# KumarRobotics/top_down_renderer

Hardware: AMD Instinct MI355X
Metric: particle-updates/sec (render+score+resample) (higher is better)
Workload: dtype f32

## Files before the change

### include/tdr.h

```cpp
#ifndef TDR_H_
#define TDR_H_

#include <stddef.h>
#include <stdint.h>

#ifdef __cplusplus
extern "C" {
#endif

#define TDR_OK 0
#define TDR_ERR_ARG (-1)
#define TDR_ERR_HIP (-2)
#define TDR_ERR_NOMEM (-3)

#define TDR_MAX_CLASSES 15
#define TDR_ST_FIELDS 7
enum { TDR_ST_INIT_X = 0, TDR_ST_INIT_Y = 1, TDR_ST_DX = 2, TDR_ST_DY = 3, TDR_ST_THETA = 4, TDR_ST_SCALE = 5,
       TDR_ST_HAVE_INIT = 6 };

typedef struct tdr_state {
  float init_x_px, init_y_px, dx_m, dy_m, theta, scale;
  uint8_t have_init;
  uint8_t pad_[3];
} tdr_state;
// ... 191 lines not shown
                          int64_t src_shard, float* dst, int64_t dst_cap, const float* info, float* out12, void* stream);

int tdr_config_compact(int on);
int tdr_config_shift_uniform(int mode);
float tdr_config_shift_uniform_span(float cells);
int tdr_config_ray_split(int k);
int tdr_config_cart_skip(int on);
int tdr_config_init_mfma(int on);
int tdr_config_uw_waves(int on);
int64_t tdr_shift_uniform_launches(void);

int tdr_profile_enable(int on);
int tdr_profile_score_ms(double* total_ms, int64_t* launches);
int tdr_profile_shares(double* dense_ms, double* scattered_ms, int64_t* scattered_particles);
int tdr_profile_variants(int64_t out[16]);

int64_t tdr_config_tuning(const char* name, int64_t value);
int tdr_su_tail_plan(int nchunks, int k, int q, int row, int* group, int* s0, int* s1);
size_t tdr_k_su_order_workspace_ints(int64_t n, int nb);
int64_t tdr_k_su_order_slots(int64_t n, int nb);
int tdr_k_su_order(const float* st, int64_t cap, int64_t n, const int32_t* perm, int nb, float span, int32_t* workspace,
                   int32_t* slots_out, int32_t* keys_out, int32_t* counts_out, int* bucket_out, void* stream);
int tdr_k_score_prep(const tdr_map_desc* map, const float* tab, const float* scan_pk, int nb, int nr, float res,
                     const float* st, int64_t cap, int64_t n, int64_t n_total, const int32_t* perm, float uniform_scale,
                     float span, float* workspace, tdr_score_ctx* ctx, int64_t* layout, void* const* out, void* stream);
int tdr_selftest_score(void);
int tdr_k_selftest_round(const float* x, int64_t n, float limit, int32_t* out, void* stream);
int tdr_libm_variant(void);
int tdr_libm_force_variant(int variant);
int tdr_sincosf_host(const float* x, int64_t n, int variant, float* sin_out, float* cos_out);
// ... 307 lines not shown
```

### top_down_renderer_amd/_lib.py

```python
import ctypes as C
import os

_PKG = os.path.dirname(os.path.abspath(__file__))
SO_PATH = os.environ.get("TDR_LIB_PATH") or os.path.join(_PKG, "libtdr_hip.so")

TDR_ST_FIELDS = 7
TDR_MAX_CLASSES = 15
TDR_SVG_NO_KEY = 0xFFFFFFFF


class FilterParamsC(C.Structure):
    _fields_ = [
        ("pos_cov", C.c_float), ("theta_cov", C.c_float), ("regularization", C.c_float),
        ("init_pos_px_x", C.c_float), ("init_pos_px_y", C.c_float), ("init_pos_px_cov", C.c_float),
        ("init_pos_m_x", C.c_float), ("init_pos_m_y", C.c_float),
        ("init_pos_deg_theta", C.c_float), ("init_pos_deg_cov", C.c_float),
        ("force_on_map", C.c_int32),
        ("fixed_scale", C.c_float), ("scale_log_min", C.c_float), ("scale_log_max", C.c_float),
        ("num_classes", C.c_int32),
        ("class_weights", C.c_float * 16),
    ]


class MapDescC(C.Structure):
# ... 142 lines not shown
    "tdr_rng_set_state_host": (_i, [_vp, _vp]),
    "tdr_k_resample_dev": (_i, [_vp, _i64, _i64, _vp, _i64, _i64, _vp, _vp]),
    "tdr_score_ctx_create": (_i, [C.POINTER(_vp)]),
    "tdr_score_ctx_destroy": (None, [_vp]),
    "tdr_score_ctx_span": (C.c_float, [_vp]),
    "tdr_score_ctx_trial_calls": (_i64, [_vp]),
    "tdr_config_tuning": (_i64, [C.c_char_p, _i64]),
    "tdr_su_tail_plan": (_i, [_i, _i, _i, _i, C.POINTER(_i), C.POINTER(_i), C.POINTER(_i)]),
    "tdr_k_su_order_workspace_ints": (C.c_size_t, [_i64, _i]),
    "tdr_k_su_order_slots": (_i64, [_i64, _i]),
    "tdr_k_su_order": (_i, [_vp, _i64, _i64, _vp, _i, _f, _vp, _vp, _vp, _vp, C.POINTER(_i), _vp]),
    "tdr_k_score_prep": (_i, [_vp, _vp, _vp, _i, _i, _f, _vp, _i64, _i64, _i64, _vp, _f, _f, _vp, _vp, C.POINTER(_i64),
                              C.POINTER(_vp), _vp]),
    "tdr_selftest_score": (_i, []),
    "tdr_profile_variants": (_i, [C.POINTER(_i64)]),
    "tdr_score_ctx_set_polar_factors": (_i, [_vp, _vp, _i, _i]),
    "tdr_polar_factors_host": (_i, [_i, _i, _f, _f, _vp]),
    "tdr_k_score_polar_ctx": (_i, [C.POINTER(MapDescC), _vp, _vp, _i, _i, _f, C.POINTER(FilterParamsC), _vp, _i64, _i64,
                                   _i64, _vp, _f, _i, _vp, _vp, _vp, _vp]),
    "tdr_score_geo_workspace_floats": (C.c_size_t, [_i, _i, _i, _i64, _i64]),
    "tdr_k_score_polar_geo": (_i, [C.POINTER(MapDescC), C.POINTER(MapDescC), _vp, _vp, _vp, _f, _f, _i, _i, _f,
                                   C.POINTER(FilterParamsC), _vp, _i64, _i64, _i64, _vp, _f, _i, _vp, _vp, _vp]),
    "tdr_score_cart_workspace_floats": (C.c_size_t, [_i, _i, _i, _i64, _i64]),
    "tdr_k_score_cart": (_i, [C.POINTER(MapDescC), _vp, _i, _i, _f, C.POINTER(FilterParamsC), _vp, _i64, _i64, _i64,
                              _vp, _vp, _vp, _vp]),
    "tdr_score_cart_init_workspace_floats": (C.c_size_t, [_i, _i, _i, _i64, _i64]),
    "tdr_k_score_cart_init": (_i, [C.POINTER(MapDescC), _vp, _i, _i, _f, C.POINTER(FilterParamsC), _vp, _i64, _i64, _i64,
                                   _vp, _vp]),
    "tdr_k_propagate": (_i, [_vp, _i64, _i64, _vp, _f, _f, _f, _i, _f, _f, _vp, _u64, _u64, _i64, _vp]),
    "tdr_rng_create": (_vp, [_u32]),
# ... 195 lines not shown
```

### top_down_renderer_amd/csrc/tdr_common.h

```cpp
#ifndef TDR_COMMON_H_
#define TDR_COMMON_H_
#include <hip/hip_runtime.h>

#include <cmath>
#include <cstdarg>
#include <cstdint>
#include <cstdio>
#include <cstdlib>
#include <cstring>
#include <limits>
#include <type_traits>
#include <utility>
#include <vector>

#include "tdr.h"
#include "tdr_config.h"
#include "tdr_internal.h"

#ifndef TDR_SCORE_U
#define TDR_SCORE_U 4
#endif
#ifndef TDR_INIT_SCAN_LDS
#define TDR_INIT_SCAN_LDS 1
#endif
// ... 43 lines not shown
#define INI_TILE 2048
#define INI_MAX_TILES 2048
int tdr_chain_total(const float* raw, const float* mean_dev, int kind, int64_t n, float* total_out, void* workspace,
                    bool have_sums, hipStream_t st);
struct UwExact {
  float sum, mean, bsum, pad;
};
int tdr_uw_chunk_pass1(const float* raw, int64_t n, void* workspace, int* cnt_valid, hipStream_t st);
int tdr_uw_chunk_pass2(const float* raw, int64_t n, UwExact* ex, const int* cnt_valid, void* workspace, int* cnt_under,
                       hipStream_t st);
int tdr_uw_small(const float* raw, const float* last_dist, int64_t n, float* w, float* info, hipStream_t st);
int tdr_mt_raw_stream(const uint32_t* state, int64_t nblocks, uint32_t* raw, hipStream_t s);
int tdr_mt_advance(const uint32_t* raw, int64_t nblocks, const uint32_t* consumed, uint32_t* state, hipStream_t s);
__host__ __device__ inline bool tdr_has_kslot(int ncls, int rf) { return ncls + 2 <= rf; }
uint32_t* tdr_profile_stats_ptr();
#endif
```

### top_down_renderer_amd/csrc/tdr_score.hip

```cpp

#include "tdr_common.h"
#include "tdr_batch.h"
#include "tdr_sincosf.h"

struct ScoreArgs {
  const float* rec;
  int rows, cols;
  float resolution;
  const float* tab;
  const float* utab = nullptr;
  const float* scan_pk;
  int nb, nr;
  float res;
  const float* st;
  int64_t cap, n;
  const int32_t* order;
  const int32_t* count = nullptr;
  const int32_t* slot_base = nullptr;
  int use_theta_override = 0;
  float theta_override = 0.f;
  int only_uninit = 0;
  int group, nchunks;
  int64_t npad;
  float* part;
// ... 770 lines not shown
  if (!g_variant_stats) {
    if (hipMalloc((void**)&g_variant_stats, 16 * sizeof(uint32_t)) != hipSuccess) { g_variant_stats = nullptr; return nullptr; }
    (void)hipMemset(g_variant_stats, 0, 16 * sizeof(uint32_t));
  }
  return g_variant_stats;
}
extern "C" int tdr_profile_variants(int64_t out[16]) {
  if (!out) return fail(TDR_ERR_ARG, "profile_variants: null pointer");
  for (int k = 0; k < 16; k++) out[k] = 0;
  if (!g_variant_stats) return TDR_OK;
  uint32_t h[16];
  HIP_TRY(hipDeviceSynchronize());
  HIP_TRY(hipMemcpy(h, g_variant_stats, sizeof(h), hipMemcpyDeviceToHost));
  HIP_TRY(hipMemset(g_variant_stats, 0, sizeof(h)));
  for (int k = 0; k < 16; k++) out[k] = h[k];
  return TDR_OK;
}
extern "C" int tdr_profile_enable(int on) {
  g_prof_on = on != 0;
  g_prof_variants = on == 2;
  g_prof_used = 0;
  g_share_valid = false;
  return TDR_OK;
}
extern "C" int tdr_profile_shares(double* dense_ms, double* scattered_ms, int64_t* scattered_particles) {
  if (!dense_ms || !scattered_ms || !scattered_particles) return fail(TDR_ERR_ARG, "profile_shares: null pointer");
  if (!g_share_valid || !g_share_counts) return fail(TDR_ERR_ARG, "profile_shares: no integer-form launch was profiled");
  float ms[2] = {0.f, 0.f};
  for (int k = 0; k < 2; k++) {
    HIP_TRY(hipEventSynchronize(g_share_ev[k][1]));
// ... 592 lines not shown
```

### top_down_renderer_amd/csrc/tdr_score_ray.hip

```cpp
#include "tdr_score_dev.h"
#include "tdr_score_su.h"

int64_t tdr_ray_padded_samples(int nb, int nr) { return (int64_t)nb * ray_blocks(nr, false) * ray_gq(nr, false) * 64; }

struct RayArgs {
  const uint32_t* crec;
  unsigned planes_off;
  unsigned plane_bytes;
  unsigned cmask_off;
  int pkcol;
  const uint32_t* dict_int;
  int dict_n;
  int rows, cols;
  float resolution;
  const float* tab;
  const float* tab_ray;
  const float* fac;
  const float* rad_ray;
  float uscale;
  const uint16_t* desc_ray;
  const uint32_t* list;
  const int32_t* n_list;
  const float* scan_pk;
  int rf, ncls, nb, nr, blocks;
  float res;
  const float* st;
  int64_t cap;
  const int32_t* slots;
  const int32_t* counts;
  const int32_t* inexact;
  int nsplit;
  int64_t npad;
  uint32_t* part;
};

template <int GQ, bool USCALE, bool FAC, bool BM, bool PATCH>
__device__ __forceinline__ void ray_body(const RayArgs& a, unsigned long long* lacc, uint32_t* ldict, uint4* lut, float2* ldir) {
  static_assert(!BM || GQ == 1, "block-major: one step per row");
  static_assert(!PATCH || BM, "the patch order is a block-major order");
  const int nsparse = a.counts[1];
  if ((int64_t)blockIdx.x * 4 >= (int64_t)nsparse * a.nsplit) return;
  const int lane = threadIdx.x & 63, wave = __builtin_amdgcn_readfirstlane(threadIdx.x >> 6);
  for (int t = threadIdx.x; t < a.dict_n; t += 256) ldict[t] = a.dict_int[t];
  if constexpr (PATCH && FAC)
    for (int t = threadIdx.x; t < a.nb; t += 256) ldir[t] = reinterpret_cast<const float2*>(a.fac)[t];
  const unsigned pconst = (unsigned)(a.pkcol + 16) + 128u;
  if (threadIdx.x < 16) {
    const int code = threadIdx.x;
    uint4 e;
    if (code >= 1 && code <= a.ncls) {
      e.x = a.planes_off + (unsigned)(code - 1) * a.plane_bytes + pconst;
      e.y = 0; e.z = 15; e.w = (unsigned)code * 512u;
    } else {
      e.x = a.cmask_off + pconst;
      e.y = 2; e.z = 0; e.w = 0;
    }
    lut[code] = e;
  }
  unsigned long long* const my = lacc + (size_t)wave * (a.ncls + 1) * 64 + lane;
  for (int c = 0; c <= a.ncls; c++) my[c * 64] = 0;
  __syncthreads();
  const int64_t gw = (int64_t)blockIdx.x * 4 + wave;
  const int64_t q = gw / a.nsplit;
  const int part_id = (int)(gw - q * a.nsplit);
  if (q >= nsparse) return;
  const int64_t slot = (int64_t)a.counts[0] + q;
  const int64_t p = a.slots[slot];
  const float scale = a.st[TDR_ST_SCALE * a.cap + p];
  const float fscale = USCALE ? a.uscale : scale;
  const float cx = a.st[TDR_ST_DX * a.cap + p] * scale + a.st[TDR_ST_INIT_X * a.cap + p];
  const float cy = a.st[TDR_ST_DY * a.cap + p] * scale + a.st[TDR_ST_INIT_Y * a.cap + p];
  const float off0 = cy / a.resolution;
  const float off1 = cx / a.resolution;
  const int shift = rot_shift_dev(a.st[TDR_ST_THETA * a.cap + p], a.nb);
  const float rmaxf = (float)a.rows, cmaxf = (float)a.cols;
  const char* __restrict__ crecb = reinterpret_cast<const char*>(a.crec);
  typedef float tdr_v2f __attribute__((ext_vector_type(2)));
  const tdr_v2f offv = {off0, off1};
  auto cell = [&](float tx, float ty, int& ri, int& ci) {
    tdr_v2f pv = {tx, ty};
// ... 82 lines not shown
    }
    uint32_t v[N * GQ], shb[N * GQ], cnt[N * GQ], acc_at[N * GQ];
#pragma unroll
    for (int u = 0; u < N; u++)
#pragma unroll
      for (int g = 0; g < GQ; g++) {
        const int s = u * GQ + g;
        int ri, ci;
        if constexpr (FAC) cell_fac(dir[u], rr_[u][g], ri, ci);
        else cell(tt[u][2 * g], tt[u][2 * g + 1], ri, ci);
        issue(dd[u][g], ri, ci, v[s], shb[s], cnt[s], acc_at[s]);
      }
#pragma unroll
    for (int s = 0; s < N * GQ; s++) consume(v[s], shb[s], cnt[s], acc_at[s]);
  };
  if constexpr (PATCH) {
    const int ngroups = a.nb / RAY_PG, sectors_all = a.blocks * ngroups;
    const int sper = (sectors_all + a.nsplit - 1) / a.nsplit;
    const int s0 = part_id * sper, s1 = min(sectors_all, s0 + sper);
    const int pl_d = lane >> 4, pl_r = lane & (RAY_PR - 1);
    const uint2* __restrict__ descq = reinterpret_cast<const uint2*>(a.desc_ray);
    float rad4[4] = {0.f, 0.f, 0.f, 0.f};
    int cur_seg = -1;
    int seg = s0 / ngroups, pg = s0 - seg * ngroups;
    for (int sc = s0; sc < s1; sc++) {
      if (seg != cur_seg) {
        cur_seg = seg;
#pragma unroll
        for (int qq = 0; qq < 4; qq++) {
          const int j = (seg * 4 + qq) * RAY_PR + pl_r;
          rad4[qq] = j < a.nr ? a.fac[2 * a.nb + j] : 1.0e30f;
        }
      }
      int wi[4];
      tdr_v2f wdir[4];
#pragma unroll
      for (int k = 0; k < 4; k++) {
        int i = pg * RAY_PG + 4 * k + pl_d - shift;
        i += i < 0 ? a.nb : 0;
        wi[k] = i;
        if constexpr (FAC) {
          const float2 dv = ldir[i];
          wdir[k] = (tdr_v2f){dv.x, dv.y};
        }
      }
#pragma unroll
      for (int h = 0; h < 2; h++) {
        uint2 dd[2];
#pragma unroll
        for (int u = 0; u < 2; u++) dd[u] = descq[((int64_t)(seg * 4 + 2 * h + u) * ngroups + pg) * 64 + lane];
        uint32_t v[8], shb[8], cnt[8], acc_at[8];
#pragma unroll
        for (int u = 0; u < 2; u++)
#pragma unroll
          for (int k = 0; k < 4; k++) {
            int ri, ci;
            if constexpr (FAC) {
              cell_fac(wdir[k], rad4[2 * h + u], ri, ci);
            } else {
              const int j = min((seg * 4 + 2 * h + u) * RAY_PR + pl_r, a.nr - 1);
              const int64_t kk = (int64_t)j * a.nb + wi[k];
              if ((seg * 4 + 2 * h + u) * RAY_PR + pl_r < a.nr) cell(a.tab[2 * kk], a.tab[2 * kk + 1], ri, ci);
              else cell(-1.0e30f, -1.0e30f, ri, ci);
            }
            const uint32_t w = k < 2 ? dd[u].x : dd[u].y;
            issue((k & 1) ? (w >> 16) : (w & 0xFFFFu), ri, ci, v[u * 4 + k], shb[u * 4 + k], cnt[u * 4 + k], acc_at[u * 4 + k]);
          }
#pragma unroll
        for (int t = 0; t < 8; t++) consume(v[t], shb[t], cnt[t], acc_at[t]);
      }
      pg++;
      if (pg == ngroups) { pg = 0; seg++; }
    }
  } else {
// ... 15 lines not shown
      cell(a.tab[2 * k], a.tab[2 * k + 1], ri, ci);
      const unsigned cell_off = plane_offset(ri, ci, a.pkcol, (int)(a.planes_off + pconst));
      uint32_t kbit = 0;
      for (int c = 0; c < a.ncls; c++) {
        const float s = a.scan_pk[bin * a.rf + c];
        if (s != 0.f) {
          const uint32_t vv = *reinterpret_cast<const uint16_t*>(crecb + cell_off + (unsigned)c * a.plane_bytes);
          kbit = vv >> 15;
          __hip_atomic_fetch_add(&my[(c + 1) * 64], (unsigned long long)(uint32_t)s * ldict[(vv & 0xFFCu) >> 2],
                                 __ATOMIC_RELAXED, __HIP_MEMORY_SCOPE_WORKGROUP);
        }
      }
      norm += (uint32_t)a.scan_pk[bin * a.rf + a.rf - 1] & (0u - kbit);
    }
  }
  uint32_t* o = a.part + (int64_t)part_id * (2 * a.ncls + 2) * a.npad + slot;
  for (int c = 0; c < a.ncls; c++) {
    unsigned long long s = __hip_atomic_load(&my[(c + 1) * 64], __ATOMIC_RELAXED, __HIP_MEMORY_SCOPE_WORKGROUP);
#pragma unroll
    for (int dlt = 32; dlt > 0; dlt >>= 1) s += __shfl_xor(s, dlt, 64);
    if (lane == 0) {
      o[(int64_t)(2 * c) * a.npad] = (uint32_t)s;
      o[(int64_t)(2 * c + 1) * a.npad] = (uint32_t)(s >> 32);
    }
  }
#pragma unroll
  for (int dlt = 32; dlt > 0; dlt >>= 1) {
    known += __shfl_xor(known, dlt, 64);
    norm += __shfl_xor(norm, dlt, 64);
  }
  if (lane == 0) {
    o[(int64_t)(2 * a.ncls) * a.npad] = norm;
    o[(int64_t)(2 * a.ncls + 1) * a.npad] = known;
  }
}
TDR_TL_BUFFER(g_timeline_ray, tdr_debug_read_timeline_ray)
template <int GQ, bool USCALE, bool BM = false, bool PATCH = false>
__global__ __launch_bounds__(256) void score_polar_ray_kernel(RayArgs a) {
  extern __shared__ unsigned long long lacc[];
  __shared__ uint32_t ldict[TDR_CMAP_MAX_DICT];
  __shared__ uint4 lut[16];
  __shared__ float2 ldir[PATCH ? RAY_PATCH_MAX_NB : 1];
  if (int_form_off(a.inexact)) return;
#ifdef TDR_SCORE_TIMELINE
  if ((int64_t)blockIdx.x * 4 >= (int64_t)a.counts[1] * a.nsplit) return;
#endif
  TDR_TL_BEGIN(g_timeline_ray)
  if (a.fac && a.inexact[2] == 0) ray_body<GQ, USCALE, true, BM, PATCH>(a, lacc, ldict, lut, ldir);
  else ray_body<GQ, USCALE, false, BM, PATCH>(a, lacc, ldict, lut, ldir);
  TDR_TL_END(g_timeline_ray)
}



bool tdr_ray_map_ok(const tdr_map_desc* map) {
  return map->crec && map->dict && map->cwords == tdr_cmap_words(map->ncls) && map->dict_n > 0 &&
         map->dict_n <= TDR_CMAP_MAX_DICT && tdr_cmap_plane_words(map->ncls, map->rows, map->cols) != 0;
}
int tdr_ray_splits(int nb, int nr, int64_t n, bool bm) {
  if (tdr_cfg().ray_split > 0) return tdr_cfg().ray_split;
  const int64_t rows = (int64_t)nb * ray_blocks(nr, bm);
  int s = 1;
  while (s < TDR_RAY_MAX_SPLIT && n * s < 32768 && rows / (2 * s) >= 8) s *= 2;
  if (s == 1 && rows >= 128) s = 2;
// ... 21 lines not shown
  r.fac = L.fac;
  r.rad_ray = reinterpret_cast<const float*>(base + W.ray_rad);
  r.uscale = L.uscale;
  r.desc_ray = reinterpret_cast<const uint16_t*>(base + W.ray_desc);
  r.list = reinterpret_cast<const uint32_t*>(base + W.ray_multi);
  r.n_list = ints + 3;
  r.scan_pk = L.scan_pk;
  r.rf = L.rf; r.ncls = map->ncls; r.nb = L.nb; r.nr = L.nr; r.blocks = ray_blocks(L.nr, ray_bm(L)); r.res = L.res;
  r.st = L.st; r.cap = L.cap;
  r.slots = base + W.slots;
  r.counts = ints;
  r.inexact = ints + 4;
  r.nsplit = L.ray_split;
  r.npad = L.npad;
  r.part = reinterpret_cast<uint32_t*>(L.part);
  const dim3 grid((unsigned)cdiv(L.n * r.nsplit, 4)), block(256);
  const size_t lds = (size_t)4 * (map->ncls + 1) * 64 * sizeof(unsigned long long);
#define TDR_LAUNCH_RAY(GQ)                                                                            \
  if (L.uniform_scale) hipLaunchKernelGGL((score_polar_ray_kernel<GQ, true>), grid, block, lds, s, r); \
  else hipLaunchKernelGGL((score_polar_ray_kernel<GQ, false>), grid, block, lds, s, r);
  if (ray_patch(L)) {
    if (L.uniform_scale) hipLaunchKernelGGL((score_polar_ray_kernel<1, true, true, true>), grid, block, lds, s, r);
    else hipLaunchKernelGGL((score_polar_ray_kernel<1, false, true, true>), grid, block, lds, s, r);
  } else if (ray_bm(L)) {
    if (L.uniform_scale) hipLaunchKernelGGL((score_polar_ray_kernel<1, true, true>), grid, block, lds, s, r);
    else hipLaunchKernelGGL((score_polar_ray_kernel<1, false, true>), grid, block, lds, s, r);
  } else switch (ray_gq(L.nr, false)) {
    case 1: TDR_LAUNCH_RAY(1) break;
    case 2: TDR_LAUNCH_RAY(2) break;
    default: TDR_LAUNCH_RAY(4) break;
  }
#undef TDR_LAUNCH_RAY
// ... 4 lines not shown
```

### top_down_renderer_amd/csrc/tdr_score_su.h

```cpp
#ifndef TDR_SCORE_SU_H_
#define TDR_SCORE_SU_H_
#include "tdr_common.h"

static inline int64_t su_npad(int64_t n, int nb) { return cdiv(n + 63 * std::min<int64_t>(nb, n), 64) * 64; }
bool tdr_su_shape_ok(int nb, int nr, int group, int64_t n_total);
struct SuWs {
  int64_t tab_su, desc, bbox, keys_in, keys_out, vals_in, vals_out, ints, slots, sort_tmp, ray_tab, ray_desc, ray_multi, ray_rad, total;
  int64_t seg_hist;
};
#define TDR_SU_TAIL_INTS 10
#define TDR_RAY_MAX_SPLIT 8
SuWs tdr_su_ws(int nb, int nr, int group, int64_t n);

#define TDR_SU_NSECT 8
__host__ __device__ static inline int su_tail_plan(int nchunks, int k, int q, int row, int* group, int* s0, int* s1) {
  const int lq = q >= 8 ? 3 : (q >= 4 ? 2 : (q >= 2 ? 1 : 0));
  const int kk = k < 0 ? 0 : (k > nchunks ? nchunks : k);
  const int head = nchunks - kk, rows = head + (kk << lq);
  if (row < 0 || row >= rows) return rows;
  if (row < head) {
    *group = row; *s0 = 0; *s1 = TDR_SU_NSECT;
  } else {
    const int t = row - head, part = t & ((1 << lq) - 1);
    *group = head + (t >> lq);
// ... 39 lines not shown
  float best = 16.f;
  float round_best = 16.f, best_ms = 3.0e38f;
  hipEvent_t e0 = nullptr, e1 = nullptr;
  bool open = false, pending = false;
  int64_t trial_calls = 0;
};
float tdr_su_span_begin(SpanTuner* t, int64_t shape, hipStream_t s);
void tdr_su_span_end(SpanTuner* t, hipStream_t s);
int tdr_su_score(const SuLaunch& L, const SuWs& W, hipStream_t s);
bool tdr_ray_map_ok(const tdr_map_desc* map);
int64_t tdr_ray_padded_samples(int nb, int nr);
int tdr_ray_splits(int nb, int nr, int64_t n, bool block_major = false);
#define RAY_PR 16
#define RAY_PG 16
#define RAY_PATCH_MAX_NB 256
static inline bool ray_bm(const SuLaunch& L) { return tdr_cfg().ray_block_major && L.fac != nullptr; }
static inline bool ray_patch(const SuLaunch& L) { return ray_bm(L) && tdr_cfg().ray_patch && L.nb % RAY_PG == 0 && L.nb <= RAY_PATCH_MAX_NB; }
static inline int ray_gq(int nr, bool bm) { return bm ? 1 : (nr <= 64 ? 1 : (nr <= 128 ? 2 : 4)); }
static inline int ray_blocks(int nr, bool bm) { return (int)cdiv(nr, 64 * ray_gq(nr, bm)); }
int tdr_ray_score(const SuLaunch& L, const SuWs& W, hipStream_t s);
#endif
```

### top_down_renderer_amd/csrc/tdr_score_su.hip

```cpp
#include <rocprim/device/device_radix_sort.hpp>

#include <atomic>

#include "tdr_score_dev.h"
#include "tdr_score_su.h"
#include "tdr_score_su_asm.h"

#define SU_CODE_FULL 0xFFu
#define SU_CODE_FULL_ALL 0xFEu
#define SU_CODE_PAD 0xFDu
#define SU_NSECT TDR_SU_NSECT
#define SU_BOX_WORDS 4096

struct SuArgs {
  const uint32_t* crec;
  const uint32_t* kmask;
  int kcolw;
  unsigned kmask_off;
  const uint32_t* dict_int;
  int dict_n, ctiles_r;
  int pkcol;
  const int32_t* inexact;
  int rows, cols;
  float resolution;
// ... 24 lines not shown
  unsigned pbase, plane_bytes;
  const float* dict;
  int dict_n;
  float* tab_su;
  uint32_t* desc;
  float* bbox;
  int gq, blocks, bm, patch, borrow;
  const uint32_t* dict_tail;
  const float* fac;
  float* tab_ray;
  float* rad_ray;
  uint16_t* desc_ray;
  uint32_t* list;
  int32_t* n_list;
  int32_t* inexact;
};
__device__ __forceinline__ void atomic_min_float(float* at, float v) {
  if (!(v == v)) return;
  if (__float_as_int(v) >= 0) atomicMin(reinterpret_cast<int*>(at), __float_as_int(v));
  else atomicMax(reinterpret_cast<unsigned*>(at), __float_as_uint(v));
}
__device__ __forceinline__ void atomic_max_float(float* at, float v) {
  if (!(v == v)) return;
  if (__float_as_int(v) >= 0) atomicMax(reinterpret_cast<int*>(at), __float_as_int(v));
  else atomicMin(reinterpret_cast<unsigned*>(at), __float_as_uint(v));
}
#define PREP_DIRS 8
__device__ __forceinline__ void score_prep_body(const PrepArgs& a, const unsigned block) {
  const int nb = a.nb, nr = a.nr, rf = a.rf, rp = a.rp;
  __shared__ float red[PREP_DIRS][64][4];
  __shared__ unsigned wg_mass, wg_listed, wg_list_base;
  if (threadIdx.x == 0) { wg_mass = 0; wg_listed = 0; }
  bool bad = false;
  for (int k = threadIdx.x; k < a.dict_n; k += blockDim.x) bad |= !(fabsf(a.dict[k]) <= 3.402823466e+38f);
  const bool dict_bad = __syncthreads_or(bad);
  if (block == 0 && threadIdx.x == 0 && a.dict_tail[1] != 1u) atomicOr(a.inexact, 1);
  const int segs = rp >> 6, lane = threadIdx.x & 63, wave = threadIdx.x >> 6;
  const int i_raw = (int)(block / segs) * PREP_DIRS + wave, j = (int)(block % segs) * 64 + lane;
  const bool live = i_raw < nb;
  const int i = live ? i_raw : nb - 1;
  const bool real = live && j < nr;
  const int64_t k = (int64_t)(j < nr ? j : nr - 1) * nb + i;
  const float2 te = *reinterpret_cast<const float2*>(a.tab + 2 * k);
  float tx = te.x, ty = te.y;
  if (a.utab) {
    tx = (tx * a.uscale) * a.res;
    ty = (ty * a.uscale) * a.res;
// ... 68 lines not shown
  bool listed = false;
  unsigned list_rank = 0;
  if (real) {
    if (a.fac) {
      float fx = a.fac[2 * i] * a.fac[2 * nb + j], fy = a.fac[2 * i + 1] * a.fac[2 * nb + j];
      if (a.uscale > 0.f) {
        fx = (fx * a.uscale) * a.res;
        fy = (fy * a.uscale) * a.res;
      }
      if (__float_as_uint(fx) != __float_as_uint(tx) || __float_as_uint(fy) != __float_as_uint(ty)) atomicOr(a.inexact + 2, 1);
    }
    if (!whole) atomicOr(a.inexact, 1);
    else if (nz == 1 && vfirst < 4096.f) d = (uint32_t)vfirst | ((uint32_t)(first + 1) << 12);
    else if (nz >= 1) { listed = true; list_rank = atomicAdd(&wg_listed, 1u); }
  }
  {
    const uint32_t own = d >> 12;
    const int ql = lane & 3;
    uint32_t c4[4];
#pragma unroll
    for (int q = 0; q < 4; q++) c4[q] = __shfl(own, (lane & 60) + q, 64);
    if (a.borrow && own == 0) {
      uint32_t pick = 0;
#pragma unroll
      for (int dist = 3; dist >= 1; dist--) {
        if (ql + dist < 4 && c4[(ql + dist) & 3]) pick = c4[(ql + dist) & 3];
        if (ql - dist >= 0 && c4[(ql - dist) & 3]) pick = c4[(ql - dist) & 3];
      }
      d = pick << 12;
    }
  }
  __syncthreads();
  if (threadIdx.x == 0) {
    if (wg_mass && (uint64_t)atomicAdd(reinterpret_cast<unsigned*>(a.inexact) + 1, wg_mass) + wg_mass >= (1u << 24)) atomicOr(a.inexact, 1);
    wg_list_base = wg_listed ? (unsigned)atomicAdd(a.n_list, (int)wg_listed) : 0u;
  }
  if (real && (lane == 0 || jj == 0)) {
    const int sect = sector(i);
    if (wave == 0 || sector(i - 1) != sect) {
      float lo0 = red[wave][lane][0], hi0 = red[wave][lane][1], lo1 = red[wave][lane][2], hi1 = red[wave][lane][3];
      for (int w = wave + 1; w < PREP_DIRS && i + (w - wave) < nb && sector(i + (w - wave)) == sect; w++) {
        lo0 = fminf(lo0, red[w][lane][0]); hi0 = fmaxf(hi0, red[w][lane][1]);
        lo1 = fminf(lo1, red[w][lane][2]); hi1 = fmaxf(hi1, red[w][lane][3]);
      }
      float* box = a.bbox + ((int64_t)chunk * SU_NSECT + sect) * 4;
      atomic_min_float(box, lo0);
      atomic_max_float(box + 1, hi0);
      atomic_min_float(box + 2, lo1);
      atomic_max_float(box + 3, hi1);
    }
  }
  __syncthreads();
  if (listed) a.list[wg_list_base + list_rank] = ((uint32_t)i << 16) | (uint32_t)j;
  if (!ray_live) return;
  const int g = j >> 6, l = j & 63, b = g / a.gq, gq = a.gq;
  const int64_t at = a.bm ? ((int64_t)b * nb + i) * 64 + l : (((int64_t)i * a.blocks + b) * 64 + l) * gq + (g - b * gq);
  int64_t at_d = at;
  if (a.patch) at_d = ((((int64_t)(j / RAY_PR) * (nb / RAY_PG) + i / RAY_PG) * 64 + (i & 3) * RAY_PR + (j % RAY_PR)) << 2) + ((i % RAY_PG) >> 2);
  if (a.fac && i == 0) a.rad_ray[((int64_t)b * 64 + l) * gq + (g - b * gq)] = real ? a.fac[2 * nb + j] : 1.0e30f;
  *reinterpret_cast<float2*>(a.tab_ray + 2 * at) = real ? make_float2(tx, ty) : make_float2(-1.0e30f, -1.0e30f);
  a.desc_ray[at_d] = (uint16_t)d;
}
__global__ __launch_bounds__(64 * PREP_DIRS) void score_prep_kernel(PrepArgs a) { score_prep_body(a, blockIdx.x); }

__global__ __launch_bounds__(256) void su_key_kernel(const float* __restrict__ st, int64_t cap, int64_t n,
                                                     const int32_t* __restrict__ perm, int nb, float span, int per_block,
                                                     uint32_t* __restrict__ keys, int32_t* __restrict__ vals,
                                                     int* __restrict__ cnt, int* __restrict__ seg_hist) {
  extern __shared__ int hist[];
  for (int k = threadIdx.x; k <= nb; k += 256) hist[k] = 0;
  __syncthreads();
  for (int it = 0; it < per_block; it += 256) {
    const int64_t t = (int64_t)blockIdx.x * per_block + it + threadIdx.x;
    if (t >= n) break;
    const int32_t p = perm ? perm[t] : (int32_t)t;
    uint32_t key = (uint32_t)rot_shift_dev(st[TDR_ST_THETA * cap + p], nb);
    if (span > 0.f) {
      auto centre = [&](int64_t q, float& x, float& y) {
// ... 737 lines not shown
  w.desc = take(4 * nbins);
  w.bbox = take(nchunks * SU_NSECT * 4);
  w.keys_in = take(n);
  w.keys_out = take(n);
  w.vals_in = take(n);
  w.vals_out = take(n);
  w.ints = take(3 * ((int64_t)nb + 1) + TDR_SU_TAIL_INTS);
  w.slots = take(su_npad(n, nb));
  w.sort_tmp = take((int64_t)((su_sort_tmp_bytes(n) + 3) / 4));
  const int64_t T = tdr_ray_padded_samples(nb, nr);
  w.ray_tab = take(2 * T);
  w.ray_desc = take((T + 1) / 2);
  w.ray_multi = take((int64_t)nb * nr);
  w.ray_rad = take(T / nb);
  w.seg_hist = take(su_seg_table_reserve(nb, n));
  w.total = o;
  return w;
}

int tdr_su_order(const SuLaunch& L, const SuWs& W, hipStream_t s, const int32_t** slots_out, const int32_t** counts_out,
                 float* box_init, int box_count) {
  int32_t* base = L.ws;
  uint32_t* keys_in = reinterpret_cast<uint32_t*>(base + W.keys_in);
  uint32_t* keys_out = reinterpret_cast<uint32_t*>(base + W.keys_out);
  int32_t* vals_in = base + W.vals_in;
  int32_t* vals_out = base + W.vals_out;
  int* cnt = base + W.ints;
  const int nkeys = L.nb + 1;
  int* start = cnt + nkeys;
  int* slot_start = start + nkeys;
// ... 88 lines not shown
            (unsigned)(plane_trows(L.map->rows) * 128) + 128u;
  p.dict = L.map->dict; p.dict_n = L.map->dict_n;
  p.tab_su = reinterpret_cast<float*>(base + W.tab_su);
  p.desc = reinterpret_cast<uint32_t*>(base + W.desc);
  p.bbox = bbox;
  const bool bm = ray_bm(L);
  p.gq = ray_gq(L.nr, bm); p.blocks = ray_blocks(L.nr, bm); p.bm = bm ? 1 : 0; p.patch = ray_patch(L) ? 1 : 0;
  p.borrow = tdr_cfg().ray_borrow ? 1 : 0;
  p.dict_tail = reinterpret_cast<const uint32_t*>(L.map->dict) + 2 * TDR_CMAP_MAX_DICT;
  p.fac = L.fac;
  p.tab_ray = reinterpret_cast<float*>(base + W.ray_tab);
  p.rad_ray = reinterpret_cast<float*>(base + W.ray_rad);
  p.desc_ray = reinterpret_cast<uint16_t*>(base + W.ray_desc);
  p.list = reinterpret_cast<uint32_t*>(base + W.ray_multi);
  p.n_list = ints + 3; p.inexact = ints + 4;
  hipLaunchKernelGGL(score_prep_kernel, dim3((unsigned)(cdiv(L.nb, PREP_DIRS) * (p.rp / 64))), dim3(64 * PREP_DIRS), 0, s, p);
  LAUNCH_CHECK("score_prep");
  return TDR_OK;
}
int tdr_su_prep_copy_out(const SuLaunch& L, const SuWs& W, hipStream_t s, int64_t layout[16], void* const out[9]) {
  const bool bm = ray_bm(L);
  const int64_t nbins = (int64_t)L.nchunks * L.nb * L.group, T = tdr_ray_padded_samples(L.nb, L.nr);
  if (layout) {
    const int64_t v[16] = {L.group, L.nchunks, prep_padded_rings(L), ray_gq(L.nr, bm), ray_blocks(L.nr, bm), bm ? 1 : 0,
                           ray_patch(L) ? 1 : 0, T, nbins, SU_NSECT, TDR_SU_TAIL_INTS, L.uniform_scale ? 1 : 0, 0, 0, 0, 0};
    for (int k = 0; k < 16; k++) layout[k] = v[k];
  }
  if (!out || !L.ws) return TDR_OK;
  const int32_t* base = L.ws;
  const struct { const void* src; size_t bytes; } parts[9] = {
      {L.uniform_scale ? L.utab_out : nullptr, sizeof(float) * 2 * (size_t)L.nb * L.nr},
// ... 57 lines not shown
```

Baseline: 24.20 million.

## Compact per-sector ray sample lists and early-exit gate in patch ray scoring

The score-prep kernel now builds, per 16-direction by 64-ring sector, compacted sample lists sorted by class code, split into single-class samples and mixed samples, along with a count table. In the patch+fac path, the ray kernel walks these lists instead of a dense grid, so empty samples are skipped. It also adds a majority 'known' gate that skips or stops the mixed-sample pass once the outcome is settled, sharing partial counts across split waves through LDS atomics and a barrier. The cost is extra prep work, more workspace and LDS, more per-sample indirection and sync, and new optional profiling counters.

```diff
diff --git a/include/tdr.h b/include/tdr.h
--- a/include/tdr.h
+++ b/include/tdr.h
@@ -229,6 +229,7 @@
 int tdr_profile_score_ms(double* total_ms, int64_t* launches);
 int tdr_profile_shares(double* dense_ms, double* scattered_ms, int64_t* scattered_particles);
 int tdr_profile_variants(int64_t out[16]);
+int tdr_profile_ray_gate(int64_t out[4]);
 
 int64_t tdr_config_tuning(const char* name, int64_t value);
 int tdr_su_tail_plan(int nchunks, int k, int q, int row, int* group, int* s0, int* s1);
diff --git a/top_down_renderer_amd/_lib.py b/top_down_renderer_amd/_lib.py
--- a/top_down_renderer_amd/_lib.py
+++ b/top_down_renderer_amd/_lib.py
@@ -180,6 +180,7 @@
                               C.POINTER(_vp), _vp]),
     "tdr_selftest_score": (_i, []),
     "tdr_profile_variants": (_i, [C.POINTER(_i64)]),
+    "tdr_profile_ray_gate": (_i, [C.POINTER(_i64)]),
     "tdr_score_ctx_set_polar_factors": (_i, [_vp, _vp, _i, _i]),
     "tdr_polar_factors_host": (_i, [_i, _i, _f, _f, _vp]),
     "tdr_k_score_polar_ctx": (_i, [C.POINTER(MapDescC), _vp, _vp, _i, _i, _f, C.POINTER(FilterParamsC), _vp, _i64, _i64,
diff --git a/top_down_renderer_amd/csrc/tdr_common.h b/top_down_renderer_amd/csrc/tdr_common.h
--- a/top_down_renderer_amd/csrc/tdr_common.h
+++ b/top_down_renderer_amd/csrc/tdr_common.h
@@ -81,4 +81,5 @@
 int tdr_mt_advance(const uint32_t* raw, int64_t nblocks, const uint32_t* consumed, uint32_t* state, hipStream_t s);
 __host__ __device__ inline bool tdr_has_kslot(int ncls, int rf) { return ncls + 2 <= rf; }
 uint32_t* tdr_profile_stats_ptr();
+uint32_t* tdr_profile_gate_ptr();
 #endif
diff --git a/top_down_renderer_amd/csrc/tdr_score.hip b/top_down_renderer_amd/csrc/tdr_score.hip
--- a/top_down_renderer_amd/csrc/tdr_score.hip
+++ b/top_down_renderer_amd/csrc/tdr_score.hip
@@ -808,6 +808,26 @@
   HIP_TRY(hipMemcpy(h, g_variant_stats, sizeof(h), hipMemcpyDeviceToHost));
   HIP_TRY(hipMemset(g_variant_stats, 0, sizeof(h)));
   for (int k = 0; k < 16; k++) out[k] = h[k];
+  return TDR_OK;
+}
+static uint32_t* g_gate_stats = nullptr;
+uint32_t* tdr_profile_gate_ptr() {
+  if (!g_prof_on || !g_prof_variants) return nullptr;
+  if (!g_gate_stats) {
+    if (hipMalloc((void**)&g_gate_stats, 4 * sizeof(uint32_t)) != hipSuccess) { g_gate_stats = nullptr; return nullptr; }
+    (void)hipMemset(g_gate_stats, 0, 4 * sizeof(uint32_t));
+  }
+  return g_gate_stats;
+}
+extern "C" int tdr_profile_ray_gate(int64_t out[4]) {
+  if (!out) return fail(TDR_ERR_ARG, "profile_ray_gate: null pointer");
+  for (int k = 0; k < 4; k++) out[k] = 0;
+  if (!g_gate_stats) return TDR_OK;
+  uint32_t h[4];
+  HIP_TRY(hipDeviceSynchronize());
+  HIP_TRY(hipMemcpy(h, g_gate_stats, sizeof(h), hipMemcpyDeviceToHost));
+  HIP_TRY(hipMemset(g_gate_stats, 0, sizeof(h)));
+  for (int k = 0; k < 4; k++) out[k] = h[k];
   return TDR_OK;
 }
 extern "C" int tdr_profile_enable(int on) {
diff --git a/top_down_renderer_amd/csrc/tdr_score_ray.hip b/top_down_renderer_amd/csrc/tdr_score_ray.hip
--- a/top_down_renderer_amd/csrc/tdr_score_ray.hip
+++ b/top_down_renderer_amd/csrc/tdr_score_ray.hip
@@ -32,18 +32,42 @@
   int nsplit;
   int64_t npad;
   uint32_t* part;
+  const uint32_t* clist;
+  const int32_t* ctab;
+  uint32_t* gate_ctr;
 };
 
+template <int N>
+__device__ __forceinline__ void ray_list_load(const uint4* __restrict__ lst, int e0, int lane, uint32_t (&w)[N]) {
+  uint4 q[(N + 3) / 4];
+#pragma unroll
+  for (int b = 0; b < (N + 3) / 4; b++) q[b] = lst[((e0 >> 8) + b) * 64 + lane];
+#pragma unroll
+  for (int u = 0; u < N; u++) {
+    const uint4 qq = q[u >> 2];
+    w[u] = (u & 3) == 0 ? qq.x : ((u & 3) == 1 ? qq.y : ((u & 3) == 2 ? qq.z : qq.w));
+  }
+}
 template <int GQ, bool USCALE, bool FAC, bool BM, bool PATCH>
-__device__ __forceinline__ void ray_body(const RayArgs& a, unsigned long long* lacc, uint32_t* ldict, uint4* lut, float2* ldir) {
+__device__ __forceinline__ void ray_body(const RayArgs& a, unsigned long long* lacc, uint32_t* ldict, uint4* lut, float2* ldir,
+                                         uint32_t (*lgate)[4]) {
   static_assert(!BM || GQ == 1, "block-major: one step per row");
   static_assert(!PATCH || BM, "the patch order is a block-major order");
+  constexpr bool COMPACT = PATCH && FAC;
   const int nsparse = a.counts[1];
   if ((int64_t)blockIdx.x * 4 >= (int64_t)nsparse * a.nsplit) return;
   const int lane = threadIdx.x & 63, wave = __builtin_amdgcn_readfirstlane(threadIdx.x >> 6);
   for (int t = threadIdx.x; t < a.dict_n; t += 256) ldict[t] = a.dict_int[t];
-  if constexpr (PATCH && FAC)
-    for (int t = threadIdx.x; t < a.nb; t += 256) ldir[t] = reinterpret_cast<const float2*>(a.fac)[t];
+  float* const lrad = reinterpret_cast<float*>(lacc + (size_t)4 * (a.ncls + 1) * 64);
+  const bool gate_shared = COMPACT && 4 % a.nsplit == 0 && (int64_t)a.nb * a.nr < (1 << 24);
+  if constexpr (COMPACT) {
+    for (int t = threadIdx.x; t < 2 * a.nb + RAY_PG; t += 256) ldir[t] = reinterpret_cast<const float2*>(a.fac)[t % a.nb];
+    for (int t = threadIdx.x; t < a.blocks * 65; t += 256) {
+      const int sg = t / 65, rr = t - sg * 65, jr = sg * 64 + rr;
+      lrad[t] = rr < 64 && jr < a.nr ? a.fac[2 * a.nb + jr] : 1.0e30f;
+    }
+    if (threadIdx.x < 16) lgate[threadIdx.x >> 2][threadIdx.x & 3] = 0;
+  }
   const unsigned pconst = (unsigned)(a.pkcol + 16) + 128u;
   if (threadIdx.x < 16) {
     const int code = threadIdx.x;
@@ -63,7 +87,10 @@
   const int64_t gw = (int64_t)blockIdx.x * 4 + wave;
   const int64_t q = gw / a.nsplit;
   const int part_id = (int)(gw - q * a.nsplit);
-  if (q >= nsparse) return;
+  if (q >= nsparse) {
+    if (COMPACT && gate_shared && a.nsplit > 1) __syncthreads();
+    return;
+  }
   const int64_t slot = (int64_t)a.counts[0] + q;
   const int64_t p = a.slots[slot];
   const float scale = a.st[TDR_ST_SCALE * a.cap + p];
@@ -176,35 +203,74 @@
 #pragma unroll
     for (int s = 0; s < N * GQ; s++) consume(v[s], shb[s], cnt[s], acc_at[s]);
   };
-  if constexpr (PATCH) {
+  uint32_t nb_mine = 0;
+  if constexpr (COMPACT) {
+    const int ngroups = a.nb / RAY_PG, sectors_all = a.blocks * ngroups;
+    const int sper = (sectors_all + a.nsplit - 1) / a.nsplit;
+    const int s0 = part_id * sper, s1 = min(sectors_all, s0 + sper);
+    int seg = s0 / ngroups, pg = s0 - seg * ngroups;
+    int4 tn = s0 < s1 ? *reinterpret_cast<const int4*>(a.ctab + (int64_t)s0 * 16 + 12) : make_int4(0, 0, 0, 0);
+    for (int sc = s0; sc < s1; sc++) {
+      const int n_a = tn.x + tn.y;
+      nb_mine += (uint32_t)(tn.z + tn.w);
+      tn = *reinterpret_cast<const int4*>(a.ctab + (int64_t)min(sc + 1, s1 - 1) * 16 + 12);
+      const uint4* __restrict__ lst = reinterpret_cast<const uint4*>(a.clist + (int64_t)sc * RAY_CL_WORDS);
+      const int dbase = (pg * RAY_PG - shift + a.nb) * 8, rbase = seg * 65 * 4;
+      const unsigned pbase_a = a.planes_off + pconst - a.plane_bytes;
+      auto step_a = [&](auto cnt_c, int e0) {
+        constexpr int N = decltype(cnt_c)::value;
+        uint32_t w[N], v[N];
+        ray_list_load<N>(lst, e0, lane, w);
+#pragma unroll
+        for (int u = 0; u < N; u++) {
+          const float2 dv = *reinterpret_cast<const float2*>(reinterpret_cast<const char*>(ldir) + dbase + (w[u] >> 25));
+          const float rad = *reinterpret_cast<const float*>(reinterpret_cast<const char*>(lrad) + rbase + ((w[u] >> 16) & 0x1FFu));
+          int ri, ci;
+          cell_fac((tdr_v2f){dv.x, dv.y}, rad, ri, ci);
+          const unsigned off = plane_offset(ri, ci, a.pkcol, (int)(pbase_a + ((w[u] >> 12) & 0xFu) * a.plane_bytes));
+          v[u] = *reinterpret_cast<const uint16_t*>(crecb + off);
+        }
+#pragma unroll
+        for (int u = 0; u < N; u++) {
+          const uint32_t kbit = v[u] >> 15, cnt = w[u] & 0xFFFu;
+          known += kbit;
+          norm = __umul24(cnt, kbit) + norm;
+          const uint32_t D = *reinterpret_cast<const uint32_t*>(reinterpret_cast<const char*>(ldict) + (v[u] & 0xFFCu));
+          unsigned long long* const acc = reinterpret_cast<unsigned long long*>(reinterpret_cast<char*>(my) + ((w[u] >> 3) & 0x1E00u));
+          __hip_atomic_fetch_add(acc, (unsigned long long)cnt * D, __ATOMIC_RELAXED, __HIP_MEMORY_SCOPE_WORKGROUP);
+        }
+      };
+      int e = 0, left = (n_a + 63) >> 6;
+      if (left > 12) { step_a(std::integral_constant<int, 8>{}, 0); e = 512; left -= 8; }
+      else if (left > 8) { step_a(std::integral_constant<int, 4>{}, 0); e = 256; left -= 4; }
+      switch (left) {
+        case 8: step_a(std::integral_constant<int, 8>{}, e); break;
+        case 7: step_a(std::integral_constant<int, 7>{}, e); break;
+        case 6: step_a(std::integral_constant<int, 6>{}, e); break;
+        case 5: step_a(std::integral_constant<int, 5>{}, e); break;
+        case 4: step_a(std::integral_constant<int, 4>{}, e); break;
+        case 3: step_a(std::integral_constant<int, 3>{}, e); break;
+        case 2: step_a(std::integral_constant<int, 2>{}, e); break;
+        case 1: step_a(std::integral_constant<int, 1>{}, e); break;
+        default: break;
+      }
+      pg++;
+      if (pg == ngroups) { pg = 0; seg++; }
+    }
+  } else if constexpr (PATCH) {
     const int ngroups = a.nb / RAY_PG, sectors_all = a.blocks * ngroups;
     const int sper = (sectors_all + a.nsplit - 1) / a.nsplit;
     const int s0 = part_id * sper, s1 = min(sectors_all, s0 + sper);
     const int pl_d = lane >> 4, pl_r = lane & (RAY_PR - 1);
     const uint2* __restrict__ descq = reinterpret_cast<const uint2*>(a.desc_ray);
-    float rad4[4] = {0.f, 0.f, 0.f, 0.f};
-    int cur_seg = -1;
     int seg = s0 / ngroups, pg = s0 - seg * ngroups;
     for (int sc = s0; sc < s1; sc++) {
-      if (seg != cur_seg) {
-        cur_seg = seg;
-#pragma unroll
-        for (int qq = 0; qq < 4; qq++) {
-          const int j = (seg * 4 + qq) * RAY_PR + pl_r;
-          rad4[qq] = j < a.nr ? a.fac[2 * a.nb + j] : 1.0e30f;
-        }
-      }
       int wi[4];
-      tdr_v2f wdir[4];
 #pragma unroll
       for (int k = 0; k < 4; k++) {
         int i = pg * RAY_PG + 4 * k + pl_d - shift;
         i += i < 0 ? a.nb : 0;
         wi[k] = i;
-        if constexpr (FAC) {
-          const float2 dv = ldir[i];
-          wdir[k] = (tdr_v2f){dv.x, dv.y};
-        }
       }
 #pragma unroll
       for (int h = 0; h < 2; h++) {
@@ -217,9 +283,7 @@
 #pragma unroll
           for (int k = 0; k < 4; k++) {
             int ri, ci;
-            if constexpr (FAC) {
-              cell_fac(wdir[k], rad4[2 * h + u], ri, ci);
-            } else {
+            {
               const int j = min((seg * 4 + 2 * h + u) * RAY_PR + pl_r, a.nr - 1);
               const int64_t kk = (int64_t)j * a.nb + wi[k];
               if ((seg * 4 + 2 * h + u) * RAY_PR + pl_r < a.nr) cell(a.tab[2 * kk], a.tab[2 * kk + 1], ri, ci);
@@ -265,6 +329,89 @@
       norm += (uint32_t)a.scan_pk[bin * a.rf + a.rf - 1] & (0u - kbit);
     }
   }
+  if constexpr (COMPACT) {
+#pragma unroll
+    for (int dlt = 32; dlt > 0; dlt >>= 1) known += __shfl_xor(known, dlt, 64);
+    const uint32_t P = (uint32_t)((int64_t)a.nb * a.nr);
+    uint32_t* const g = lgate[gate_shared ? wave - part_id : 0];
+    uint32_t tot_a = known, nb_all = nb_mine;
+    if (gate_shared && a.nsplit > 1) {
+      if (lane == 0) {
+        atomicAdd(&g[0], known);
+        atomicAdd(&g[1], nb_mine);
+      }
+      __syncthreads();
+      tot_a = *reinterpret_cast<volatile uint32_t*>(&g[0]);
+      nb_all = *reinterpret_cast<volatile uint32_t*>(&g[1]);
+    }
+    const bool settled = gate_shared && (2 * tot_a >= P || 2 * (tot_a + nb_all) < P);
+    uint32_t known_b = 0, blocks_b = 0;
+    bool early = false;
+    if (!settled) {
+      const int ngroups = a.nb / RAY_PG, sectors_all = a.blocks * ngroups;
+      const int sper = (sectors_all + a.nsplit - 1) / a.nsplit;
+      const int s0 = part_id * sper, s1 = min(sectors_all, s0 + sper);
+      int seg = s0 / ngroups, pg = s0 - seg * ngroups;
+      const uint4 em = lut[0];
+      for (int sc = s0; sc < s1 && !early; sc++) {
+        const int32_t* __restrict__ tb = a.ctab + (int64_t)sc * 16;
+        const int n_a = tb[12] + tb[13], n_b = tb[14] + tb[15];
+        const uint4* __restrict__ lst = reinterpret_cast<const uint4*>(a.clist + (int64_t)sc * RAY_CL_WORDS + ((n_a + 255) >> 8) * 256);
+        const int dbase = (pg * RAY_PG - shift + a.nb) * 8, rbase = seg * 65 * 4;
+        auto step_b = [&](auto cnt_c, int e0) {
+          constexpr int N = decltype(cnt_c)::value;
+          uint32_t w[N], v[N], shb[N];
+          ray_list_load<N>(lst, e0, lane, w);
+#pragma unroll
+          for (int u = 0; u < N; u++) {
+            const float2 dv = *reinterpret_cast<const float2*>(reinterpret_cast<const char*>(ldir) + dbase + (w[u] >> 25));
+            const float rad = *reinterpret_cast<const float*>(reinterpret_cast<const char*>(lrad) + rbase + ((w[u] >> 16) & 0x1FFu));
+            int ri, ci;
+            cell_fac((tdr_v2f){dv.x, dv.y}, rad, ri, ci);
+            const unsigned off = plane_offset(ri >> (int)em.y, ci >> (int)em.y, a.pkcol, (int)em.x);
+            shb[u] = (((uint32_t)ri & 3u) << 2) | ((uint32_t)ci & 3u);
+            v[u] = *reinterpret_cast<const uint16_t*>(crecb + off);
+          }
+          uint32_t c = 0;
+#pragma unroll
+          for (int u = 0; u < N; u++) c += (uint32_t)__popcll(__ballot((v[u] >> shb[u]) & 1u));
+          return c;
+        };
+        for (int e = 0; e < n_b && !early; e += 256) {
+          const int left = (n_b - e + 63) >> 6;
+          uint32_t c = 0;
+          if (left >= 4) c = step_b(std::integral_constant<int, 4>{}, e);
+          else if (left == 3) c = step_b(std::integral_constant<int, 3>{}, e);
+          else if (left == 2) c = step_b(std::integral_constant<int, 2>{}, e);
+          else c = step_b(std::integral_constant<int, 1>{}, e);
+          known_b += c;
+          blocks_b++;
+          if (gate_shared) {
+            uint32_t tot_b = known_b;
+            if (a.nsplit > 1) {
+              uint32_t old = 0;
+              if (lane == 0) old = atomicAdd(&g[2], c);
+              tot_b = (uint32_t)__builtin_amdgcn_readfirstlane((int)old) + c;
+            }
+            early = 2 * (tot_a + tot_b) >= P && (e + 256 < n_b || sc + 1 < s1);
+          }
+        }
+        pg++;
+        if (pg == ngroups) { pg = 0; seg++; }
+      }
+      known += known_b;
+    }
+    if (a.gate_ctr && lane == 0) {
+      if (blocks_b) atomicAdd(&a.gate_ctr[3], blocks_b);
+      if (!gate_shared) {
+        if (part_id == 0) atomicAdd(&a.gate_ctr[2], 1u);
+      } else {
+        const uint32_t mine = 1u + (settled ? 0u : 0x100u) + (early ? 0x10000u : 0u);
+        const uint32_t all = atomicAdd(&g[3], mine) + mine;
+        if ((all & 0xFFu) == (uint32_t)a.nsplit) atomicAdd(&a.gate_ctr[(all >> 16) ? 1 : ((all & 0xFF00u) ? 2 : 0)], 1u);
+      }
+    }
+  }
   uint32_t* o = a.part + (int64_t)part_id * (2 * a.ncls + 2) * a.npad + slot;
   for (int c = 0; c < a.ncls; c++) {
     unsigned long long s = __hip_atomic_load(&my[(c + 1) * 64], __ATOMIC_RELAXED, __HIP_MEMORY_SCOPE_WORKGROUP);
@@ -277,7 +424,7 @@
   }
 #pragma unroll
   for (int dlt = 32; dlt > 0; dlt >>= 1) {
-    known += __shfl_xor(known, dlt, 64);
+    if constexpr (!COMPACT) known += __shfl_xor(known, dlt, 64);
     norm += __shfl_xor(norm, dlt, 64);
   }
   if (lane == 0) {
@@ -291,14 +438,15 @@
   extern __shared__ unsigned long long lacc[];
   __shared__ uint32_t ldict[TDR_CMAP_MAX_DICT];
   __shared__ uint4 lut[16];
-  __shared__ float2 ldir[PATCH ? RAY_PATCH_MAX_NB : 1];
+  __shared__ float2 ldir[PATCH ? 2 * RAY_PATCH_MAX_NB + RAY_PG : 1];
+  __shared__ uint32_t lgate[4][4];
   if (int_form_off(a.inexact)) return;
 #ifdef TDR_SCORE_TIMELINE
   if ((int64_t)blockIdx.x * 4 >= (int64_t)a.counts[1] * a.nsplit) return;
 #endif
   TDR_TL_BEGIN(g_timeline_ray)
-  if (a.fac && a.inexact[2] == 0) ray_body<GQ, USCALE, true, BM, PATCH>(a, lacc, ldict, lut, ldir);
-  else ray_body<GQ, USCALE, false, BM, PATCH>(a, lacc, ldict, lut, ldir);
+  if (a.fac && a.inexact[2] == 0) ray_body<GQ, USCALE, true, BM, PATCH>(a, lacc, ldict, lut, ldir, lgate);
+  else ray_body<GQ, USCALE, false, BM, PATCH>(a, lacc, ldict, lut, ldir, lgate);
   TDR_TL_END(g_timeline_ray)
 }
 
@@ -350,8 +498,11 @@
   r.nsplit = L.ray_split;
   r.npad = L.npad;
   r.part = reinterpret_cast<uint32_t*>(L.part);
+  r.clist = reinterpret_cast<const uint32_t*>(base + W.ray_clist);
+  r.ctab = base + W.ray_ctab;
+  r.gate_ctr = ray_patch(L) ? tdr_profile_gate_ptr() : nullptr;
   const dim3 grid((unsigned)cdiv(L.n * r.nsplit, 4)), block(256);
-  const size_t lds = (size_t)4 * (map->ncls + 1) * 64 * sizeof(unsigned long long);
+  const size_t lds = (size_t)4 * (map->ncls + 1) * 64 * sizeof(unsigned long long) + (ray_patch(L) ? (size_t)r.blocks * 65 * sizeof(float) : 0);
 #define TDR_LAUNCH_RAY(GQ)                                                                            \
   if (L.uniform_scale) hipLaunchKernelGGL((score_polar_ray_kernel<GQ, true>), grid, block, lds, s, r); \
   else hipLaunchKernelGGL((score_polar_ray_kernel<GQ, false>), grid, block, lds, s, r);
diff --git a/top_down_renderer_amd/csrc/tdr_score_su.h b/top_down_renderer_amd/csrc/tdr_score_su.h
--- a/top_down_renderer_amd/csrc/tdr_score_su.h
+++ b/top_down_renderer_amd/csrc/tdr_score_su.h
@@ -7,6 +7,7 @@
 struct SuWs {
   int64_t tab_su, desc, bbox, keys_in, keys_out, vals_in, vals_out, ints, slots, sort_tmp, ray_tab, ray_desc, ray_multi, ray_rad, total;
   int64_t seg_hist;
+  int64_t ray_clist, ray_ctab;
 };
 #define TDR_SU_TAIL_INTS 10
 #define TDR_RAY_MAX_SPLIT 8
@@ -77,6 +78,8 @@
 #define RAY_PR 16
 #define RAY_PG 16
 #define RAY_PATCH_MAX_NB 256
+#define RAY_CL_WORDS 1280
+#define RAY_CL_NONE 0x01001000u
 static inline bool ray_bm(const SuLaunch& L) { return tdr_cfg().ray_block_major && L.fac != nullptr; }
 static inline bool ray_patch(const SuLaunch& L) { return ray_bm(L) && tdr_cfg().ray_patch && L.nb % RAY_PG == 0 && L.nb <= RAY_PATCH_MAX_NB; }
 static inline int ray_gq(int nr, bool bm) { return bm ? 1 : (nr <= 64 ? 1 : (nr <= 128 ? 2 : 4)); }
diff --git a/top_down_renderer_amd/csrc/tdr_score_su.hip b/top_down_renderer_amd/csrc/tdr_score_su.hip
--- a/top_down_renderer_amd/csrc/tdr_score_su.hip
+++ b/top_down_renderer_amd/csrc/tdr_score_su.hip
@@ -62,6 +62,8 @@
   uint32_t* list;
   int32_t* n_list;
   int32_t* inexact;
+  uint32_t* clist;
+  int32_t* ctab;
 };
 __device__ __forceinline__ void atomic_min_float(float* at, float v) {
   if (!(v == v)) return;
@@ -73,12 +75,17 @@
   if (__float_as_int(v) >= 0) atomicMax(reinterpret_cast<int*>(at), __float_as_int(v));
   else atomicMin(reinterpret_cast<unsigned*>(at), __float_as_uint(v));
 }
-#define PREP_DIRS 8
+#define PREP_DIRS_COMPACT RAY_PG
+#define PREP_KEYS 80
+template <int PREP_DIRS>
 __device__ __forceinline__ void score_prep_body(const PrepArgs& a, const unsigned block) {
   const int nb = a.nb, nr = a.nr, rf = a.rf, rp = a.rp;
   __shared__ float red[PREP_DIRS][64][4];
   __shared__ unsigned wg_mass, wg_listed, wg_list_base;
+  __shared__ unsigned crow[PREP_DIRS == PREP_DIRS_COMPACT ? PREP_DIRS : 1][PREP_KEYS], ckeys[PREP_KEYS], cbase[PREP_KEYS];
   if (threadIdx.x == 0) { wg_mass = 0; wg_listed = 0; }
+  if constexpr (PREP_DIRS == PREP_DIRS_COMPACT)
+    for (int t = threadIdx.x; t < PREP_DIRS * PREP_KEYS; t += 64 * PREP_DIRS) (&crow[0][0])[t] = 0;
   bool bad = false;
   for (int k = threadIdx.x; k < a.dict_n; k += blockDim.x) bad |= !(fabsf(a.dict[k]) <= 3.402823466e+38f);
   const bool dict_bad = __syncthreads_or(bad);
@@ -177,6 +184,21 @@
     else if (nz == 1 && vfirst < 4096.f) d = (uint32_t)vfirst | ((uint32_t)(first + 1) << 12);
     else if (nz >= 1) { listed = true; list_rank = atomicAdd(&wg_listed, 1u); }
   }
+  const bool compact = PREP_DIRS == PREP_DIRS_COMPACT && a.clist != nullptr && j < a.blocks * 64;
+  unsigned ckey = 0, crank = 0;
+  if (compact) {
+    const unsigned unit = (unsigned)lane >> 4, code = d >> 12;
+    const unsigned long long umask = 0xFFFFull << (16 * unit), below = (1ull << lane) - 1ull;
+    ckey = code ? unit * 16u + code : 64u + unit;
+    for (unsigned c = 0; c <= (unsigned)a.ncls; c++) {
+      const unsigned long long same = __ballot(real && code == c) & umask;
+      if (real && code == c) {
+        crank = (unsigned)__popcll(same & below);
+        if ((same >> lane) == 1ull) crow[wave][ckey] = crank + 1u;
+      }
+    }
+  }
+  const uint32_t centry = (((uint32_t)i & (RAY_PG - 1)) << 28) | (((uint32_t)j & 63u) << 18) | d;
   {
     const uint32_t own = d >> 12;
     const int ql = lane & 3;
@@ -197,6 +219,23 @@
   if (threadIdx.x == 0) {
     if (wg_mass && (uint64_t)atomicAdd(reinterpret_cast<unsigned*>(a.inexact) + 1, wg_mass) + wg_mass >= (1u << 24)) atomicOr(a.inexact, 1);
     wg_list_base = wg_listed ? (unsigned)atomicAdd(a.n_list, (int)wg_listed) : 0u;
+  }
+  if (compact) {
+    if (threadIdx.x < PREP_KEYS) {
+      unsigned run = 0;
+      for (int w = 0; w < PREP_DIRS; w++) {
+        const unsigned c = crow[w][threadIdx.x];
+        crow[w][threadIdx.x] = run;
+        run += c;
+      }
+      ckeys[threadIdx.x] = run;
+    }
+    __syncthreads();
+    if (threadIdx.x < PREP_KEYS) {
+      unsigned at = 0;
+      for (int q = 0; q < (int)threadIdx.x; q++) at += ckeys[q];
+      cbase[threadIdx.x] = at;
+    }
   }
   if (real && (lane == 0 || jj == 0)) {
     const int sect = sector(i);
@@ -215,6 +254,28 @@
   }
   __syncthreads();
   if (listed) a.list[wg_list_base + list_rank] = ((uint32_t)i << 16) | (uint32_t)j;
+  if (compact) {
+    const int64_t sector = (int64_t)(j >> 6) * (nb / RAY_PG) + i / RAY_PG;
+    const unsigned n_a = cbase[64];
+    if (threadIdx.x < 512) {
+      const unsigned stream = threadIdx.x >> 8, t = threadIdx.x & 255u;
+      const unsigned n = stream ? cbase[67] + ckeys[67] - n_a : n_a, blk = (stream ? (n_a + 255u) >> 8 : 0u) + (n >> 8);
+      if (t >= (n & 255u) && (n & 255u)) a.clist[sector * RAY_CL_WORDS + blk * 256u + (t & 63u) * 4u + (t >> 6)] = RAY_CL_NONE;
+    }
+    if (real) {
+      unsigned r = cbase[ckey] + crow[wave][ckey] + crank, blk0 = 0;
+      if (ckey >= 64u) { r -= n_a; blk0 = (n_a + 255u) >> 8; }
+      a.clist[sector * RAY_CL_WORDS + (blk0 + (r >> 8)) * 256u + (r & 63u) * 4u + ((r >> 6) & 3u)] = centry;
+    }
+    if (threadIdx.x < 4) {
+      const unsigned u = threadIdx.x;
+      int32_t* t = a.ctab + sector * 16 + 4 * u;
+      t[0] = (int32_t)cbase[16 * u];
+      t[1] = (int32_t)(cbase[16 * u + 16] - cbase[16 * u]);
+      t[2] = (int32_t)(cbase[64 + u] - n_a);
+      t[3] = (int32_t)ckeys[64 + u];
+    }
+  }
   if (!ray_live) return;
   const int g = j >> 6, l = j & 63, b = g / a.gq, gq = a.gq;
   const int64_t at = a.bm ? ((int64_t)b * nb + i) * 64 + l : (((int64_t)i * a.blocks + b) * 64 + l) * gq + (g - b * gq);
@@ -224,7 +285,8 @@
   *reinterpret_cast<float2*>(a.tab_ray + 2 * at) = real ? make_float2(tx, ty) : make_float2(-1.0e30f, -1.0e30f);
   a.desc_ray[at_d] = (uint16_t)d;
 }
-__global__ __launch_bounds__(64 * PREP_DIRS) void score_prep_kernel(PrepArgs a) { score_prep_body(a, blockIdx.x); }
+template <int PREP_DIRS>
+__global__ __launch_bounds__(64 * PREP_DIRS) void score_prep_kernel(PrepArgs a) { score_prep_body<PREP_DIRS>(a, blockIdx.x); }
 
 __global__ __launch_bounds__(256) void su_key_kernel(const float* __restrict__ st, int64_t cap, int64_t n,
                                                      const int32_t* __restrict__ perm, int nb, float span, int per_block,
@@ -992,6 +1054,10 @@
   w.ray_multi = take((int64_t)nb * nr);
   w.ray_rad = take(T / nb);
   w.seg_hist = take(su_seg_table_reserve(nb, n));
+  const bool patch_shape = nb % RAY_PG == 0 && nb <= RAY_PATCH_MAX_NB;
+  const int64_t sectors = patch_shape ? (int64_t)(nb / RAY_PG) * ray_blocks(nr, true) : 0;
+  w.ray_clist = take(sectors * RAY_CL_WORDS);
+  w.ray_ctab = take(sectors * 16);
   w.total = o;
   return w;
 }
@@ -1110,7 +1176,15 @@
   p.desc_ray = reinterpret_cast<uint16_t*>(base + W.ray_desc);
   p.list = reinterpret_cast<uint32_t*>(base + W.ray_multi);
   p.n_list = ints + 3; p.inexact = ints + 4;
-  hipLaunchKernelGGL(score_prep_kernel, dim3((unsigned)(cdiv(L.nb, PREP_DIRS) * (p.rp / 64))), dim3(64 * PREP_DIRS), 0, s, p);
+  p.clist = nullptr; p.ctab = nullptr;
+  if (p.patch) {
+    p.clist = reinterpret_cast<uint32_t*>(base + W.ray_clist);
+    p.ctab = base + W.ray_ctab;
+    hipLaunchKernelGGL(score_prep_kernel<PREP_DIRS_COMPACT>, dim3((unsigned)(L.nb / PREP_DIRS_COMPACT * (p.rp / 64))),
+                       dim3(64 * PREP_DIRS_COMPACT), 0, s, p);
+  } else {
+    hipLaunchKernelGGL(score_prep_kernel<8>, dim3((unsigned)(cdiv(L.nb, 8) * (p.rp / 64))), dim3(64 * 8), 0, s, p);
+  }
   LAUNCH_CHECK("score_prep");
   return TDR_OK;
 }
```

Result: faster. 24.78 million, median of 6 (+2.4%).
